# KubiakJakub01/Blokus-RL

Measured on AMD Instinct MI355X. Metric: MCTS sims/sec on 20x20 Blokus (4 players, 256 games/GPU, 100 sims/move), higher is better.
Workload: dtype fp32 net (fp32 operands split into f16 hi+lo, 3 f16 MFMA products, f32 accumulation: fp32-class error, tests/test_leafnet_gpu.py) / f64 search / u32 bitboards; 1 GPU; config 3 (N=1) / 4 (N=8): AlphaZero self-play 20x20, 256 concurrent games per GPU, 100 sims/move, ResNet-5x64 leaf eval; global_batch=256, parallelism=dp1 (independent games), model=resnet

## Files before the change

### blokus_rl_amd/alphazero/batched_mcts.py

```python
from __future__ import annotations

import ctypes

import numpy as np
import torch

from ..engine import Engine, EngineError, _check, _ptr


_OWN_OBS = object()


class BatchedMCTS:
    def __init__(self, eng: Engine, trees: int, node_cap: int = 8192, child_cap: int | None = None):
        self.eng = eng
        self.lib = eng.lib
        self.T = trees
        self.node_cap = node_cap
        if child_cap is None:
            per_node = 256 if eng.N >= 14 else 64
            child_cap = trees * node_cap * per_node
        self.child_cap = child_cap
        h = ctypes.c_void_p()
        with torch.cuda.device(eng.device):
# ... 46 lines not shown
        assert weight.is_contiguous() and weight.shape == (self.eng.A, feat.shape[1]) and bias.shape == (self.eng.A,)
        assert values.dtype == torch.float32 and values.shape == (self.T, self.eng.P)
        sel = roots is not None
        if obs is _OWN_OBS:
            obs = self.obs
        if obs is not None:
            assert obs.dtype == torch.float32 and obs.shape == self.obs.shape and obs.device == self.obs.device
        _check(self.lib.bk_mcts_leaf_step(self.h, ctypes.c_void_p(feat.data_ptr()), feat.stride(0), feat.shape[1],
                                          _ptr(weight), _ptr(bias), _ptr(values), int(sel), _ptr(roots),
                                          _ptr(active), float(cpuct), _ptr(self.status) if sel else None,
                                          _ptr(obs) if sel else None,
                                          _ptr(self.leaf_mask) if sel and want_mask else None,
                                          self._s()))
        return (self.status, obs, self.leaf_mask) if sel else None

    @property
    def leaf_states_ptr(self) -> int:
        p = ctypes.c_void_p()
        _check(self.lib.bk_mcts_leaf_states(self.h, ctypes.byref(p)))
        return int(p.value)

    def root_policy(self, roots: torch.Tensor, active: torch.Tensor | None, temperature: float, cap: int = 2048,
                    zero: bool = True):
        alloc = torch.zeros if zero else torch.empty
        ids = alloc((self.T, cap), dtype=torch.int32, device=self.eng.device)
        pi = alloc((self.T, cap), dtype=torch.float64, device=self.eng.device)
        counts = alloc(self.T, dtype=torch.int32, device=self.eng.device)
        _check(self.lib.bk_mcts_root_policy(self.h, _ptr(roots), _ptr(active), float(temperature), _ptr(ids),
                                            _ptr(pi), cap, _ptr(counts), self._s()))
        return ids, pi, counts
# ... 49 lines not shown
```

### blokus_rl_amd/alphazero/selfplay.py

```python
from __future__ import annotations

import os
import time
from dataclasses import dataclass, field

import torch

from ..engine import Engine, _check, _ptr
from .batched_mcts import BatchedMCTS


@dataclass
class Examples:
    states: torch.Tensor
    ids: torch.Tensor
    pi: torch.Tensor
    k: torch.Tensor
    z: torch.Tensor

    def __len__(self):
        return int(self.states.shape[0])


@dataclass
# ... 90 lines not shown
            return self.const_logp, self.const_v
        if self.graph is not None:
            if obs.data_ptr() != self.static_obs.data_ptr():
                self.static_obs.copy_(obs)
            self.graph.replay()
            return self.static_lp, self.static_v
        return self._forward(obs)


class SelfPlay:
    def __init__(self, eng: Engine, model: torch.nn.Module | None, games: int, num_sims: int = 100,
                 cpuct: float = 1.0, temperature: float = 1.0, dirichlet_alpha: float = 1.0,
                 dirichlet_weight: float = 0.25, node_cap: int | None = None, child_cap: int | None = None,
                 cap: int = 2048, seed: int = 0, nn_dtype: torch.dtype = torch.float32, use_graph: bool = True,
                 continuous: bool = False, sim_graph_sims: int | None = None, record_plies: int | None = None,
                 leaf_input: str | None = None):
        self.eng = eng
        self.G = games
        self.num_sims = num_sims
        self.sim_graph_sims = (sim_graph_sims or int(os.environ.get("BK_SIM_GRAPH_SIMS", "0"))
                               or self.graph_sims_for(num_sims))
        self.cpuct = cpuct
        self.temperature = temperature
        self.alpha = dirichlet_alpha
        self.weight = dirichlet_weight
        self.cap = cap
        self.continuous = continuous
        self.record_plies = record_plies if record_plies is not None else (
            4 * self.max_game_plies(eng) if continuous else 0)
        if node_cap is None:
            node_cap = self.node_cap_for(eng, num_sims)
        self.mcts = BatchedMCTS(eng, games, node_cap=node_cap, child_cap=child_cap)
        self.evaluator = LeafEvaluator(model, eng, games, nn_dtype, use_graph)
        self._use_graph = use_graph
        mode = leaf_input if leaf_input is not None else os.environ.get("BK_LEAF_INPUT", "planes")
        if mode not in ("planes", "states"):
            raise ValueError(f"leaf_input / BK_LEAF_INPUT must be planes or states, got {mode!r}")
        self.leaf_input = mode if mode == "planes" or self.evaluator.takes_states else "planes"
        if getattr(self.evaluator, "planar", False) and self.evaluator.graph is not None:
            self.mcts.obs = self.evaluator.static_obs
        dev = eng.device
        self.gen = torch.Generator(device=dev)
        self.gen.manual_seed(seed)
        self._seed = int(seed) & 0xFFFFFFFFFFFFFFFF
        self._init_state = eng.init_states(1)
        self.roots = eng.init_states(games)
        self.active = torch.ones(games, dtype=torch.int32, device=dev)
        self.first_ply = torch.ones(games, dtype=torch.bool, device=dev)
        self.game_id = torch.arange(games, dtype=torch.int64, device=dev)
        self._stats = SelfPlayStats()
        self._next_gid = torch.full((), games, dtype=torch.int64, device=dev)
        self._sims_dev = torch.zeros((), dtype=torch.int64, device=dev)
        self._fin_dev = torch.zeros((), dtype=torch.int64, device=dev)
        self._zcap = 0
        self.z_table = torch.zeros((0, eng.P), dtype=torch.float32, device=dev)
        self.z_known = torch.zeros(0, dtype=torch.bool, device=dev)
        self._ensure_zcap()
        self._records: list[tuple[torch.Tensor, ...]] = []
        self.timers = None
        self._graph = None
        self._window: list[tuple[torch.Tensor, ...]] = []
        self._dropped_plies = 0
        self._cap_overflow = torch.zeros((), dtype=torch.int32, device=dev)
        self.last_action = torch.full((games,), -1, dtype=torch.int32, device=dev)

    @staticmethod
    def max_game_plies(eng: Engine) -> int:
        return eng.num_pieces * eng.P

    @classmethod
    def node_cap_for(cls, eng: Engine, num_sims: int) -> int:
        return int(num_sims) * cls.max_game_plies(eng) + 1

    def check(self) -> dict:
        from ..engine import EngineError

        c = self.mcts.check()
        if int(self._cap_overflow.item()):
            raise EngineError(f"a root had more than cap={self.cap} children: raise SelfPlay(cap=...)")
# ... 20 lines not shown
            out, v = self.evaluator.forward_states(self.mcts.leaf_states_ptr, self.mcts.status)
        else:
            out, v = self.evaluator(obs)
        if self.evaluator.sparse:
            self.mcts.leaf_logits(out, self.evaluator.policy_w, self.evaluator.policy_b)
            return None, v, 2
        return out, v, 0

    def simulate(self):
        if self.timers is not None:
            return self._simulate_timed()
        _, obs, _ = self.mcts.select(self.roots, self.active, self.cpuct)
        logp, v, mode = self._evaluate(obs)
        self.mcts.expand_backup(logp, v, prior_mode=mode)


    @staticmethod
    def graph_sims_for(num_sims: int) -> int:
        if num_sims <= 100:
            return max(num_sims, 1)
        d = max(k for k in range(1, 101) if num_sims % k == 0)
        return d if d >= 10 else 10

    def _simulations(self, n: int):
        k = self.sim_graph_sims
        if n >= k and self._graph_usable():
            g = self._sim_graph()
            self._g_roots.copy_(self.roots)
            self._g_active.copy_(self.active)
            for _ in range(n // k):
                g.replay()
            n -= (n // k) * k
        for _ in range(n):
            self.simulate()

    def _graph_usable(self) -> bool:
        ev = self.evaluator
        return (self.timers is None and self._use_graph and (ev.model is None or ev.graph is not None)
                and os.environ.get("BK_SIM_GRAPH", "1") != "0")

    def _sim_body(self):
        _, obs, _ = self.mcts.select(self._g_roots, self._g_active, self.cpuct)
        ev = self.evaluator
        if ev.model is None:
            self.mcts.expand_backup(ev.const_logp, ev.const_v, prior_mode=0)
            return
        if self.leaf_input == "states":
            out, v = ev.forward_states(self.mcts.leaf_states_ptr, self.mcts.status)
        else:
            out, v = ev._forward(obs)
        if ev.sparse:
            self.mcts.leaf_logits(out, ev.policy_w, ev.policy_b)
            self.mcts.expand_backup(None, v, prior_mode=2)
        else:
            self.mcts.expand_backup(out, v, prior_mode=0)

    def _sim_graph(self):
        if self._graph is None:
            self._g_roots = self.roots.clone()
            self._g_active = self.active.clone()
            ev = self.evaluator
            g = torch.cuda.CUDAGraph()
            with torch.cuda.graph(g):
                if ev.model is not None and ev.sparse:
                    _, obs, _ = self.mcts.select(self._g_roots, self._g_active, self.cpuct)
                    states = self.leaf_input == "states"
                    for i in range(self.sim_graph_sims):
                        if states:
                            out, v = ev.forward_states(self.mcts.leaf_states_ptr, self.mcts.status)
                        else:
                            out, v = ev._forward(obs)
                        last = i == self.sim_graph_sims - 1
                        self.mcts.leaf_step(out, ev.policy_w, ev.policy_b, v, None if last else self._g_roots,
                                            self._g_active, self.cpuct, want_mask=False,
                                            obs=None if states else obs)
                else:
                    for _ in range(self.sim_graph_sims):
                        self._sim_body()
            self._graph = g
# ... 173 lines not shown
```

### blokus_rl_amd/csrc/mcts.hip

```cpp
#define BK_BOARD_SYNC() ::bk::wave_lds_sync()
#ifdef BK_STAMPS
#include <hip/hip_runtime.h>
static __device__ unsigned long long g_step_stamps[4096][16];
#define BK_MASK_STAMP(i) \
  do { if (threadIdx.x == 0 && blockIdx.x < 4096 && blockDim.x > 256) g_step_stamps[blockIdx.x][i] = __builtin_amdgcn_s_memtime(); } while (0)
#endif
#include <algorithm>
#include <cmath>
#include <cstring>
#include <vector>

#include "../../include/blokus_engine.h"
#include "ctx.h"
#include "legal_rows.h"
#include "mcts_dev.h"

namespace bk {

constexpr int kResetBlocks = 8;
__global__ __launch_bounds__(256) void k_reset(DevMcts m, const int32_t* flags) {
  const int t = blockIdx.y;
  if (flags && !flags[t]) return;
  TabEntry* tab = m.tab + (size_t)t * m.TS;
  for (int i = blockIdx.x * 256 + threadIdx.x; i < m.TS; i += kResetBlocks * 256) tab[i] = TabEntry{0ull, 0u, 0};
  if (blockIdx.x == 0 && threadIdx.x == 0) { m.tree_nodes[t] = 0; m.tree_children[t] = 0; }
}

constexpr int kSelectWaves = 4;
__global__ __launch_bounds__(64 * kSelectWaves) void k_select(DevPreset dp, DevMcts m, const uint32_t* __restrict__ roots,
                                                              const int32_t* __restrict__ active, double cpuct,
                                                              int32_t* __restrict__ status_out, float* __restrict__ obs,
                                                              uint64_t* __restrict__ mask_out, double root_eps) {
  extern __shared__ __attribute__((aligned(16))) uint32_t lds[];
  __shared__ int status_sh;
  const int wave = __builtin_amdgcn_readfirstlane(threadIdx.x >> 6);
  if (wave == 0) {
    const int st = select_descend(dp, m, blockIdx.x, roots, active, cpuct, status_out, lds, 0, nullptr, root_eps);
    if (lane_id() == 0) status_sh = st;
  }
  __syncthreads();
  select_leaf<kSelectWaves>(dp, m, blockIdx.x, status_sh, obs, mask_out, lds, wave);
}

constexpr int kLeafR = 1;
__global__ __launch_bounds__(256) void k_leaf_logits(DevPreset dp, DevMcts m, const float* __restrict__ feat,
                                                     int64_t ldf, int F, const float* __restrict__ W,
                                                     const float* __restrict__ bias) {
  extern __shared__ __attribute__((aligned(16))) uint32_t lds[];
  leaf_logits_tree<kLeafR>(dp, m, blockIdx.x, blockIdx.y, kLeafBlocks, feat, ldf, F, W, bias, lds);
}

__global__ __launch_bounds__(64) void k_expand_backup(DevPreset dp, DevMcts m, const float* __restrict__ logp,
                                                      const float* __restrict__ values, int prior_mode) {
  extern __shared__ __attribute__((aligned(16))) uint32_t lds[];
  expand_tree(dp, m, blockIdx.x, logp, values, prior_mode, lds);
}

__device__ __forceinline__ void wg_store_handoff() {
  __builtin_amdgcn_s_waitcnt(0x0F70);
  __syncthreads();
  asm volatile("buffer_inv sc0" ::: "memory");
}
constexpr int kStepWaves = 16;
__global__ __launch_bounds__(64 * kStepWaves) void k_leaf_step(DevPreset dp, DevMcts m, const float* __restrict__ feat,
                                                                 int64_t ldf, int F, const float* __restrict__ W,
                                                                 const float* __restrict__ bias,
                                                                 const float* __restrict__ values, int do_select,
                                                                 const uint32_t* __restrict__ roots,
                                                                 const int32_t* __restrict__ active, double cpuct,
                                                                 int32_t* __restrict__ status_out,
                                                                 float* __restrict__ obs,
                                                                 uint64_t* __restrict__ mask_out) {
  extern __shared__ __attribute__((aligned(16))) uint32_t lds[];
  __shared__ int status_sh;
  const int t = blockIdx.x;
  const int wave = __builtin_amdgcn_readfirstlane(threadIdx.x >> 6);
#ifdef BK_STAMPS
#define BK_STEP_STAMP(i) \
  do { if (do_select && threadIdx.x == 0 && t < 4096) g_step_stamps[t][i] = __builtin_amdgcn_s_memtime(); } while (0)
#else
#define BK_STEP_STAMP(i) do { } while (0)
#endif
  BK_STEP_STAMP(0);
  leaf_logits_tree<kLeafR>(dp, m, t, 0, 1, feat, ldf, F, W, bias, lds);
  wg_store_handoff();
  BK_STEP_STAMP(1);
  if (wave == 0) expand_tree(dp, m, t, nullptr, values, 2, lds);
  wg_store_handoff();
  BK_STEP_STAMP(2);
  if (!do_select) return;
// ... 5 lines not shown
  BK_STEP_STAMP(3);
  select_leaf<kStepWaves>(dp, m, t, status_sh, obs, mask_out, lds, wave);
  BK_STEP_STAMP(4);
#undef BK_STEP_STAMP
}

__global__ __launch_bounds__(64 * kStepWaves) void k_leaf_step_ov(DevPreset dp, DevMcts m, const float* __restrict__ feat,
                                                                    int64_t ldf, int F, const float* __restrict__ W,
                                                                    const float* __restrict__ bias,
                                                                    const float* __restrict__ values, int do_select,
                                                                    const uint32_t* __restrict__ roots,
                                                                    const int32_t* __restrict__ active, double cpuct,
                                                                    int32_t* __restrict__ status_out,
                                                                    float* __restrict__ obs,
                                                                    uint64_t* __restrict__ mask_out, int sel_off,
                                                                    int skipz) {
  extern __shared__ __attribute__((aligned(16))) uint32_t lds[];
  __shared__ int status_sh, status0_sh;
  __shared__ StepExpand sx;
  const int t = blockIdx.x;
  const int wave = __builtin_amdgcn_readfirstlane(threadIdx.x >> 6);
#ifdef BK_STAMPS
#define BK_OV_STAMP(i) \
  do { if (lane_id() == 0 && do_select && t < 4096) g_step_stamps[t][i] = __builtin_amdgcn_s_memtime(); } while (0)
#else
#define BK_OV_STAMP(i) do { } while (0)
#endif
  if (threadIdx.x == 0) {
    sx.ready = 0;
    sx.pready = 0;
    sx.done = 0;
    sx.leaf_ready = 0;
    sx.slice = 0;
    sx.loaded = 0;
    sx.counted = 0;
// ... 247 lines not shown
  if (!rc) rc = mcts_alloc(m, &d.tree_ctr, T * 8);
  if (!rc) rc = hip_check(hipMemset(d.tree_ctr, 0, T * 8 * sizeof(unsigned long long)), "memset tree counters");
  if (!rc) rc = hip_check(hipMemset(d.leaf_status, 0, T * sizeof(int32_t)), "memset status");
  if (!rc) rc = hip_check(hipMemset(d.depth, 0, T * sizeof(int32_t)), "memset depth");
  if (rc) { bk_mcts_destroy(m); return rc; }
  rc = bk_mcts_reset(m, nullptr, nullptr);
  if (!rc) rc = hip_check(hipDeviceSynchronize(), "sync");
  if (rc) { bk_mcts_destroy(m); return rc; }
  *out = m;
  return BK_OK;
}

int bk_mcts_destroy(bk_mcts* m) {
  if (!m) return BK_OK;
  for (void* p : m->allocs) (void)hipFree(p);
  delete m;
  return BK_OK;
}

int bk_mcts_reset(bk_mcts* m, const int32_t* reset_flags, void* stream) {
  BK_REQUIRE(m, "null mcts");
  hipLaunchKernelGGL(k_reset, dim3(kResetBlocks, m->d.T), dim3(256), 0, (hipStream_t)stream, m->d,
                     reset_flags);
  return launch_check("k_reset");
}

int bk_mcts_select_eps(bk_mcts* m, const void* roots, const int32_t* active, double cpuct, double root_eps,
                       int32_t* leaf_status, float* obs, uint64_t* leaf_mask, void* stream) {
  BK_REQUIRE(m && roots && leaf_status && obs, "bad argument");
  BK_REQUIRE(root_eps >= 0.0, "bk_mcts_select_eps: root_eps >= 0");
  const DevPreset& dp = m->ctx->dp;
  const size_t lds = sizeof(uint32_t) * (size_t)(kStateWords + 2 * kMaxN + dp.W32pad);
  hipLaunchKernelGGL(k_select, dim3(m->d.T), dim3(kWave * kSelectWaves), lds, (hipStream_t)stream, dp, m->d,
                     (const uint32_t*)roots, active, cpuct, leaf_status, obs, leaf_mask, root_eps);
  return launch_check("k_select");
}

int bk_mcts_select(bk_mcts* m, const void* roots, const int32_t* active, double cpuct, int32_t* leaf_status,
                   float* obs, uint64_t* leaf_mask, void* stream) {
  return bk_mcts_select_eps(m, roots, active, cpuct, 1e-6, leaf_status, obs, leaf_mask, stream);
}

int bk_mcts_leaf_logits(bk_mcts* m, const float* feat, int64_t ldf, int F, const float* W, const float* bias,
                        void* stream) {
  BK_REQUIRE(m && feat && W && bias && F > 0 && F <= kMaxFeat && ldf >= F, "bad argument");
  BK_REQUIRE(((uintptr_t)W & 15u) == 0 || (F & 3) != 0, "bk_mcts_leaf_logits: W must be 16-byte aligned");
  const DevPreset& dp = m->ctx->dp;
  const size_t lds = sizeof(uint32_t) * ((size_t)dp.W32pad + kLeafCap + F);
  hipLaunchKernelGGL(k_leaf_logits, dim3(m->d.T, kLeafBlocks), dim3(256), lds, (hipStream_t)stream, dp, m->d, feat,
                     ldf, F, W, bias);
  return launch_check("k_leaf_logits");
}

int bk_mcts_leaf_step(bk_mcts* m, const float* feat, int64_t ldf, int F, const float* W, const float* bias,
                      const float* values, int do_select, const void* roots, const int32_t* active, double cpuct,
                      int32_t* leaf_status, float* obs, uint64_t* leaf_mask, void* stream) {
  BK_REQUIRE(m && feat && W && bias && values && F > 0 && F <= kMaxFeat && ldf >= F, "bad argument");
  BK_REQUIRE(((uintptr_t)W & 15u) == 0 || (F & 3) != 0, "bk_mcts_leaf_step: W must be 16-byte aligned");
  BK_REQUIRE(!do_select || (roots && leaf_status), "bad argument: select outputs");
  const DevPreset& dp = m->ctx->dp;
  const char* ov = getenv("BK_STEP_OVERLAP");
  const int overlap = ov ? atoi(ov) : 1;
  if (overlap) {
    const int sel_off = (int)(((size_t)dp.W32pad + 2 * kLeafCap + F + 3) & ~(size_t)3);
    const size_t words = (size_t)sel_off + kStateWords + 2 * kMaxN + dp.W32pad;
    const char* sz = getenv("BK_LEAF_SKIP0");
    const int skipz = sz ? atoi(sz) : 1;
    hipLaunchKernelGGL(k_leaf_step_ov, dim3(m->d.T), dim3(kWave * kStepWaves), sizeof(uint32_t) * words,
                       (hipStream_t)stream, dp, m->d, feat, ldf, F, W, bias, values, do_select,
                       (const uint32_t*)roots, active, cpuct, leaf_status, obs, leaf_mask, sel_off, skipz);
    return launch_check("k_leaf_step_ov");
  }
  size_t words = (size_t)dp.W32pad + kLeafCap + F;
  words = std::max(words, (size_t)dp.W32pad + kExpandLdsIds);
  words = std::max(words, (size_t)(kStateWords + 2 * kMaxN + dp.W32pad));
  hipLaunchKernelGGL(k_leaf_step, dim3(m->d.T), dim3(kWave * kStepWaves), sizeof(uint32_t) * words,
                     (hipStream_t)stream, dp, m->d, feat, ldf, F, W, bias, values, do_select,
                     (const uint32_t*)roots, active, cpuct, leaf_status, obs, leaf_mask);
  return launch_check("k_leaf_step");
}

int bk_mcts_expand_backup(bk_mcts* m, const float* logp, const float* values, int prior_mode, void* stream) {
  BK_REQUIRE(m && values && (prior_mode == 0 || prior_mode == 1 || prior_mode == 2), "bad argument");
  BK_REQUIRE(logp || prior_mode == 2, "bad argument: logp");
  const DevPreset& dp = m->ctx->dp;
  const size_t lds = sizeof(uint32_t) * ((size_t)dp.W32pad + kExpandLdsIds);
  hipLaunchKernelGGL(k_expand_backup, dim3(m->d.T), dim3(kWave), lds, (hipStream_t)stream, dp, m->d, logp, values,
                     prior_mode);
  return launch_check("k_expand_backup");
}

int bk_mcts_root_policy(bk_mcts* m, const void* roots, const int32_t* active, double temperature, int32_t* ids,
                        double* pi, int cap, int32_t* counts, void* stream) {
  BK_REQUIRE(m && roots && ids && pi && counts && cap > 0 && temperature >= 0.0, "bad argument");
// ... 61 lines not shown
```

### blokus_rl_amd/csrc/mcts_dev.h

```cpp
#pragma once
#include <cmath>
#include <vector>

#include "../../include/blokus_engine.h"
#include "ctx.h"
#include "legal_rows.h"

namespace bk {

constexpr int kMaxDepth = 96;
constexpr int kExpandLdsIds = 2048;
constexpr int kGatherRegs = 16;
constexpr int kLeafCap = 2048;
constexpr int kLeafBlocks = 4;
constexpr int kMaxFeat = 2048;
constexpr int kLeafQ = 16;

#ifdef BK_STAMPS
static __device__ unsigned long long g_stamps[2][4096][8];
#define BK_STAMP(k, i) \
  do { if (lane_id() == 0 && blockIdx.x < 4096) g_stamps[k][blockIdx.x][i] = __builtin_amdgcn_s_memtime(); } while (0)
#else
#define BK_STAMP(k, i) do { } while (0)
#endif
// ... 924 lines not shown
  }
  for (int i = l + kGatherRegs * kWave; i < K; i += kWave) {
    m.ch_id[off + i] = ids[i];
    m.ch_N[off + i] = 0u;
    m.ch_Q[off + i] = 0.0;
    m.ch_P[off + i] = expf((lg[i] - mx) - lse);
  }
}

}

struct bk_mcts {
  bk_ctx* ctx = nullptr;
  bk::DevMcts d{};
  std::vector<void*> allocs;
};
```

### blokus_rl_amd/engine.py

```python
from __future__ import annotations

import ctypes
import os
from dataclasses import dataclass

import numpy as np
import torch

HERE = os.path.dirname(os.path.abspath(__file__))
LIB_PATH = os.environ.get("BK_LIB") or os.path.join(HERE, "_lib", "libblokus_hip.so")
STATE_BYTES = 384
STATE_WORDS = STATE_BYTES // 4

W_PIECES, W_HASH, W_TO_MOVE, W_PLY, W_FLAGS = 80, 84, 86, 87, 88

_vp = ctypes.c_void_p
_i = ctypes.c_int
_SIGS = {
    "bk_last_error": (ctypes.c_char_p, []),
    "bk_version": (_i, []),
    "bk_state_bytes": (_i, []),
    "bk_ctx_create": (_i, [_i, _i, _i, _i, ctypes.POINTER(_vp)]),
    "bk_ctx_destroy": (_i, [_vp]),
    "bk_action_size": (_i, [_vp]),
# ... 5 lines not shown
    "bk_legal_mask": (_i, [_vp, _vp, _vp, _i, _vp, _vp, _vp]),
    "bk_legal_ids": (_i, [_vp, _vp, _vp, _i, _vp, _i, _vp, _vp]),
    "bk_next_state": (_i, [_vp, _vp, _vp, _i, _vp, _vp, _vp, _vp]),
    "bk_game_ended": (_i, [_vp, _vp, _i, _vp, _vp, _vp]),
    "bk_observe": (_i, [_vp, _vp, _i, _vp, _vp]),
    "bk_square_counts": (_i, [_vp, _vp, _i, _vp, _vp]),
    "bk_mcts_create": (_i, [_vp, _i, _i, ctypes.c_int64, ctypes.POINTER(_vp)]),
    "bk_mcts_destroy": (_i, [_vp]),
    "bk_mcts_reset": (_i, [_vp, _vp, _vp]),
    "bk_mcts_select": (_i, [_vp, _vp, _vp, ctypes.c_double, _vp, _vp, _vp, _vp]),
    "bk_mcts_select_eps": (_i, [_vp, _vp, _vp, ctypes.c_double, ctypes.c_double, _vp, _vp, _vp, _vp]),
    "bk_mcts_expand_backup": (_i, [_vp, _vp, _vp, _i, _vp]),
    "bk_mcts_leaf_logits": (_i, [_vp, _vp, ctypes.c_int64, _i, _vp, _vp, _vp]),
    "bk_mcts_leaf_step": (_i, [_vp, _vp, ctypes.c_int64, _i, _vp, _vp, _vp, _i, _vp, _vp, ctypes.c_double, _vp,
                               _vp, _vp, _vp]),
    "bk_mcts_root_policy": (_i, [_vp, _vp, _vp, ctypes.c_double, _vp, _vp, _i, _vp, _vp]),
    "bk_mcts_root_stats": (_i, [_vp, _vp, _vp, _vp, _vp, _vp, _vp, _i, _vp, _vp]),
    "bk_mcts_counters": (_i, [_vp, _vp, _vp]),
    "bk_mcts_leaf_info": (_i, [_vp, _vp, _vp, _vp]),
    "bk_mcts_leaf_states": (_i, [_vp, ctypes.POINTER(_vp)]),
    "bk_ply_policy": (_i, [_vp, _vp, _vp, _vp, _vp, _i, _i, ctypes.c_double, ctypes.c_double, ctypes.c_uint64,
                           ctypes.c_uint64, _vp, _vp, _vp, _vp, _vp, _vp, _vp]),
    "bk_ply_finish": (_i, [_i, _i, _vp, _vp, _vp, _vp, _vp, _vp, _vp, _i, _i, _vp, _vp, _vp, _vp, _vp, _vp, _vp,
                           ctypes.c_int64, _vp, _vp, _vp, _vp, _vp]),
    "bk_vec_reset": (_i, [_vp, _vp, _vp, _vp, _i, _vp, _vp, _vp]),
    "bk_vec_step": (_i, [_vp, _vp, _vp, _vp, _i, _vp, _vp, _vp, _vp, _vp]),
    "bk_vec_policy": (_i, [_vp, _vp, _vp, _vp, _i, _i, _vp, _vp, _vp]),
    "bk_vec_step_policy": (_i, [_vp, _vp, _vp, _vp, _i, _i, _vp, _vp, _vp, _vp, _vp, _vp, _vp]),
    "bk_replay_stride": (ctypes.c_size_t, [_i]),
    "bk_replay_batch": (_i, [_vp, _vp, _i, _vp, _i, _vp, _vp, _vp, _vp, _vp, _vp, _vp]),
# ... 32 lines not shown
    "bk_resnet_stem_tower_heads": (_i, [_vp, _i, _i, _i, _vp, _vp, _i, _vp, _vp, _vp, _vp, _vp, _vp, _vp, _vp, _vp,
                                        _vp, _vp, _vp, _vp, _vp, _i, _vp, _vp, _vp]),
    "bk_leafnet_x3_weight_bytes": (_i, [_i]),
    "bk_leafnet_x3_supported": (_i, [_i]),
    "bk_leafnet_x3": (_i, [_vp, _i, _i, _i, _vp, _vp, _vp, _i, _vp, _vp, _vp, _vp] + [_vp] * 8 + [_i, _vp, _vp, _vp, _vp]),
    "bk_leafnet_x3_states": (_i, [_vp, _vp, _i, _i, _i, _vp, _vp, _vp, _i, _vp, _vp, _vp, _vp] + [_vp] * 8
                             + [_vp, _vp, _vp, _vp]),
    "bk_leafnet_w3_weight_bytes": (_i, []),
    "bk_leafnet_w3_supported": (_i, [_i]),
    "bk_leafnet_w3": (_i, [_vp, _i, _i, _i, _vp, _vp, _vp, _i, _vp, _vp, _vp, _vp] + [_vp] * 8 + [_i, _vp, _vp, _vp, _vp, _vp]),
}

_LIB = None


class EngineError(RuntimeError):
    pass


def load_library(path: str = LIB_PATH) -> ctypes.CDLL:
    global _LIB
    if _LIB is not None:
        return _LIB
    if not os.path.exists(path):
        raise EngineError(
            f"HIP engine library not built: {path}. Run `python -c 'import __graft_entry__ as g; g.build()'`."
        )
    lib = ctypes.CDLL(path)
    for name, (res, args) in _SIGS.items():
        fn = getattr(lib, name)
# ... 184 lines not shown
```

### blokus_rl_amd/nets.py

```python
from __future__ import annotations

import ctypes

import torch
import torch.nn.functional as F
from torch import nn


class NativeBatchNorm2d(nn.BatchNorm2d):

    def forward(self, x):
        self._check_input_dim(x)
        factor = 0.0 if self.momentum is None else self.momentum
        if self.training and self.track_running_stats and self.num_batches_tracked is not None:
            self.num_batches_tracked.add_(1)
            factor = 1.0 / float(self.num_batches_tracked) if self.momentum is None else self.momentum
        use_batch = self.training or (self.running_mean is None and self.running_var is None)
        track = not self.training or self.track_running_stats
        rm = self.running_mean if track else None
        rv = self.running_var if track else None
        return torch.native_batch_norm(x, self.weight, self.bias, rm, rv, use_batch, factor, self.eps)[0]


def use_native_batchnorm(model: nn.Module) -> nn.Module:
# ... 315 lines not shown
    nl = 2 * len(f.blocks)
    assert model.x3_wtower.numel() == nl * lib.bk_leafnet_x3_weight_bytes(64)
    assert model.x3_wstem.numel() == lib.bk_leafnet_x3_weight_bytes(8)
    P = f.value_fc2.out_features
    pf = torch.empty((B, 2 * N * N), dtype=torch.float32, device=dev)
    v = torch.empty((B, P), dtype=torch.float32, device=dev)
    out = torch.empty((B, 64, N, N), dtype=torch.float32, device=dev,
                      memory_format=torch.channels_last) if want_out else None
    h = model.x3_heads
    _check(lib.bk_leafnet_x3_states(
        sptr, _ptr(status), B, N, f.stem.in_channels // 2, _ptr(model.x3_wstem), _ptr(model.x3_sstem), _ptr(h[0]), nl,
        _ptr(model.x3_wtower), _ptr(model.x3_stower), _ptr(model.b_tower), _ptr(model.x3_bounds),
        *[_ptr(t) for t in h[1:]], _ptr(pf), _ptr(v),
        None if out is None else ctypes.c_void_p(out.data_ptr()), _stream(dev)))
    return (pf, v, out) if want_out else (pf, v)


_OBSERVERS: dict = {}


def _observe_states(states: torch.Tensor, N: int, P: int) -> torch.Tensor:
    from .engine import Engine

    key = (N, P, states.device)
    eng = _OBSERVERS.get(key)
    if eng is None:
        eng = _OBSERVERS[key] = Engine(N, P, 5, device=states.device)
    return eng.observe(states.contiguous())


# ... 256 lines not shown
```

### include/blokus_engine.h

```cpp
#ifndef BLOKUS_ENGINE_H
#define BLOKUS_ENGINE_H

#include <stddef.h>
#include <stdint.h>

#ifdef __cplusplus
extern "C" {
#endif

#define BK_OK 0
#define BK_EINVAL -1
#define BK_EHIP -2
#define BK_EILLEGAL -3
#define BK_ECAPACITY -4
#define BK_ENOMEM -5

#define BK_STATE_BYTES 384
#define BK_MAX_N 20
#define BK_MAX_P 4

typedef struct bk_ctx bk_ctx;
typedef struct bk_mcts bk_mcts;

const char* bk_last_error(void);
// ... 32 lines not shown

int bk_mcts_select(bk_mcts* m, const void* roots, const int32_t* active, double cpuct,
                   int32_t* leaf_status, float* obs, uint64_t* leaf_mask, void* stream);
int bk_mcts_select_eps(bk_mcts* m, const void* roots, const int32_t* active, double cpuct, double root_eps,
                       int32_t* leaf_status, float* obs, uint64_t* leaf_mask, void* stream);

int bk_mcts_expand_backup(bk_mcts* m, const float* logp, const float* values, int prior_mode,
                          void* stream);

int bk_mcts_leaf_logits(bk_mcts* m, const float* feat, int64_t ldf, int F, const float* W, const float* bias,
                        void* stream);

int bk_mcts_leaf_step(bk_mcts* m, const float* feat, int64_t ldf, int F, const float* W, const float* bias,
                      const float* values, int do_select, const void* roots, const int32_t* active, double cpuct,
                      int32_t* leaf_status, float* obs, uint64_t* leaf_mask, void* stream);

int bk_mcts_root_policy(bk_mcts* m, const void* roots, const int32_t* active, double temperature,
                        int32_t* ids, double* pi, int cap, int32_t* counts, void* stream);

int bk_mcts_root_stats(bk_mcts* m, const void* roots, const int32_t* active, int32_t* ids,
                       uint32_t* n, double* q, float* p, int cap, int32_t* counts, void* stream);

int bk_mcts_leaf_info(bk_mcts* m, void* leaf_states, int32_t* depths, void* stream);

int bk_mcts_leaf_states(bk_mcts* m, const void** states);

int bk_mcts_counters(bk_mcts* m, int64_t* out, void* stream);

int bk_ply_policy(const int32_t* ids, const double* pi, const int32_t* counts, const int32_t* active,
                  const uint8_t* first_ply, int G, int cap, double dirichlet_weight, double dirichlet_alpha,
// ... 96 lines not shown

int bk_leafnet_x3_states(const void* states, const int32_t* status, int B, int N, int P, const void* wstem,
                         const float* sstem, const float* bstem, int nlayers, const void* wtower,
                         const float* stower, const float* btower, const float* bounds, const float* wp,
                         const float* bp, const float* wv, const float* bv, const float* w1t, const float* b1,
                         const float* w2, const float* b2, float* pf, float* vout, float* out, void* stream);

int bk_leafnet_w3_weight_bytes(void);
int bk_leafnet_w3_supported(int N);
int bk_leafnet_w3(const float* obs, int B, int N, int cin, const void* wstem, const float* sstem, const float* bstem,
                  int nlayers, const void* utower, const float* stower, const float* btower, const float* bounds,
                  const float* wp, const float* bp, const float* wv, const float* bv, const float* w1t, const float* b1,
                  const float* w2, const float* b2, int P, float* pf, float* vout, float* x0ws, float* out,
                  void* stream);

#ifdef __cplusplus
}
#endif
#endif
```

Before: 1.330 million sims/s.

## Pipeline MCTS simulations across game groups on multiple streams

Splits the trees into up to four groups, each on its own HIP stream. Each group runs its own select, leaf-net and leaf-step chain, linked by ring events, so tree-search kernels of one group can overlap the network evaluation of another inside the captured graph. Kernels gain a t0 offset so they can run on a subrange of trees. This adds stream and event management and more, smaller launches. It is on by default (4 groups) when the evaluator is sparse fp32 and takes states.

New measurement: 1.442 million sims/s, median of 6. 8.4% higher.

```diff
diff --git a/blokus_rl_amd/alphazero/batched_mcts.py b/blokus_rl_amd/alphazero/batched_mcts.py
--- a/blokus_rl_amd/alphazero/batched_mcts.py
+++ b/blokus_rl_amd/alphazero/batched_mcts.py
@@ -84,6 +84,34 @@
                                           self._s()))
         return (self.status, obs, self.leaf_mask) if sel else None
 
+    def select_range(self, t0: int, n: int, roots: torch.Tensor, active: torch.Tensor | None, cpuct: float = 1.0):
+        _check(self.lib.bk_mcts_select_range(self.h, int(t0), int(n), _ptr(roots), _ptr(active), float(cpuct),
+                                             _ptr(self.status), _ptr(self.obs), _ptr(self.leaf_mask), self._s()))
+        return self.status, self.obs, self.leaf_mask
+
+    def leaf_step_range(self, t0: int, n: int, feat: torch.Tensor, weight: torch.Tensor, bias: torch.Tensor,
+                        values: torch.Tensor, roots: torch.Tensor | None = None, active: torch.Tensor | None = None,
+                        cpuct: float = 1.0):
+        assert feat.dtype == torch.float32 and feat.shape[0] == self.T and feat.stride(1) == 1
+        assert weight.is_contiguous() and weight.shape == (self.eng.A, feat.shape[1]) and bias.shape == (self.eng.A,)
+        assert values.dtype == torch.float32 and values.shape == (self.T, self.eng.P)
+        sel = roots is not None
+        _check(self.lib.bk_mcts_leaf_step_range(self.h, int(t0), int(n), ctypes.c_void_p(feat.data_ptr()),
+                                                feat.stride(0), feat.shape[1], _ptr(weight), _ptr(bias), _ptr(values),
+                                                int(sel), _ptr(roots), _ptr(active), float(cpuct),
+                                                _ptr(self.status) if sel else None, _ptr(self.obs) if sel else None,
+                                                _ptr(self.leaf_mask) if sel else None, self._s()))
+        return (self.status, self.obs, self.leaf_mask) if sel else None
+
+    def sims_pipelined(self, net_args, n_sims: int, groups: int, weight: torch.Tensor, bias: torch.Tensor,
+                       roots: torch.Tensor, active: torch.Tensor | None, cpuct: float = 1.0,
+                       obs: torch.Tensor | None = None, ring: int = 1):
+        assert weight.is_contiguous() and bias.shape == (self.eng.A,)
+        assert weight.shape == (self.eng.A, 2 * self.eng.N * self.eng.N)
+        _check(self.lib.bk_mcts_sims_pipelined(self.h, ctypes.byref(net_args), int(n_sims), int(groups), int(ring),
+                                               _ptr(weight), _ptr(bias), _ptr(roots), _ptr(active), float(cpuct),
+                                               _ptr(self.status), _ptr(obs), self._s()))
+
     @property
     def leaf_states_ptr(self) -> int:
         p = ctypes.c_void_p()
diff --git a/blokus_rl_amd/alphazero/selfplay.py b/blokus_rl_amd/alphazero/selfplay.py
--- a/blokus_rl_amd/alphazero/selfplay.py
+++ b/blokus_rl_amd/alphazero/selfplay.py
@@ -128,7 +128,8 @@
                  dirichlet_weight: float = 0.25, node_cap: int | None = None, child_cap: int | None = None,
                  cap: int = 2048, seed: int = 0, nn_dtype: torch.dtype = torch.float32, use_graph: bool = True,
                  continuous: bool = False, sim_graph_sims: int | None = None, record_plies: int | None = None,
-                 leaf_input: str | None = None):
+                 leaf_input: str | None = None, sim_groups: int | None = None, sim_ring: int | bool | None = None,
+                 sim_groups_min_games: int = 64):
         self.eng = eng
         self.G = games
         self.num_sims = num_sims
@@ -153,6 +154,17 @@
         self.leaf_input = mode if mode == "planes" or self.evaluator.takes_states else "planes"
         if getattr(self.evaluator, "planar", False) and self.evaluator.graph is not None:
             self.mcts.obs = self.evaluator.static_obs
+        k = int(sim_groups if sim_groups is not None else os.environ.get("BK_SIM_GROUPS", self.SIM_GROUPS_DEFAULT))
+        if k not in (1, 2, 4):
+            raise ValueError(f"sim_groups / BK_SIM_GROUPS must be 1, 2 or 4, got {k}")
+        ev = self.evaluator
+        pipelined = (ev.sparse and ev.dtype == torch.float32 and ev.model.takes_states()
+                     and games >= max(sim_groups_min_games, k))
+        self.sim_groups = k if pipelined else 1
+        ring = sim_ring if sim_ring is not None else os.environ.get("BK_SIM_RING")
+        self.sim_ring = int(ring) if ring is not None else (1 if self.sim_groups == 2 else 2)
+        if self.sim_ring not in (0, 1, 2):
+            raise ValueError(f"sim_ring / BK_SIM_RING must be 0, 1 or 2, got {self.sim_ring}")
         dev = eng.device
         self.gen = torch.Generator(device=dev)
         self.gen.manual_seed(seed)
@@ -173,10 +185,13 @@
         self._records: list[tuple[torch.Tensor, ...]] = []
         self.timers = None
         self._graph = None
+        self._pipe_args = None
         self._window: list[tuple[torch.Tensor, ...]] = []
         self._dropped_plies = 0
         self._cap_overflow = torch.zeros((), dtype=torch.int32, device=dev)
         self.last_action = torch.full((games,), -1, dtype=torch.int32, device=dev)
+
+    SIM_GROUPS_DEFAULT = 4
 
     @staticmethod
     def max_game_plies(eng: Engine) -> int:
@@ -227,6 +242,23 @@
         logp, v, mode = self._evaluate(obs)
         self.mcts.expand_backup(logp, v, prior_mode=mode)
 
+    def _pipelined(self, n: int, roots: torch.Tensor, active: torch.Tensor, eager: bool = False):
+        if self._pipe_args is None:
+            from ..nets import leafnet_x3_args
+
+            ev, m, N = self.evaluator, self.mcts, self.eng.N
+            states = self.leaf_input == "states"
+            pf = torch.empty((self.G, 2 * N * N), dtype=torch.float32, device=self.eng.device)
+            v = torch.empty((self.G, self.eng.P), dtype=torch.float32, device=self.eng.device)
+            args = leafnet_x3_args(ev.model, pf, v, obs=None if states else m.obs,
+                                   states=m.leaf_states_ptr if states else None, status=m.status if states else None)
+            self._pipe_args = (args, pf, v, None if states else m.obs)
+        args, _, _, obs = self._pipe_args
+        ev = self.evaluator
+        groups, ring = (min(self.sim_groups, 2), 1) if eager else (self.sim_groups, self.sim_ring)
+        self.mcts.sims_pipelined(args, n, groups, ev.policy_w, ev.policy_b, roots, active, self.cpuct, obs=obs,
+                                 ring=ring)
+
 
     @staticmethod
     def graph_sims_for(num_sims: int) -> int:
@@ -244,6 +276,9 @@
             for _ in range(n // k):
                 g.replay()
             n -= (n // k) * k
+        elif n > 0 and self.sim_groups > 1 and self.timers is None:
+            self._pipelined(n, self.roots, self.active, eager=True)
+            n = 0
         for _ in range(n):
             self.simulate()
 
@@ -273,9 +308,13 @@
             self._g_roots = self.roots.clone()
             self._g_active = self.active.clone()
             ev = self.evaluator
+            if self.sim_groups > 1:
+                self._pipelined(0, self._g_roots, self._g_active)
             g = torch.cuda.CUDAGraph()
             with torch.cuda.graph(g):
-                if ev.model is not None and ev.sparse:
+                if self.sim_groups > 1:
+                    self._pipelined(self.sim_graph_sims, self._g_roots, self._g_active)
+                elif ev.model is not None and ev.sparse:
                     _, obs, _ = self.mcts.select(self._g_roots, self._g_active, self.cpuct)
                     states = self.leaf_input == "states"
                     for i in range(self.sim_graph_sims):
diff --git a/blokus_rl_amd/csrc/mcts.hip b/blokus_rl_amd/csrc/mcts.hip
--- a/blokus_rl_amd/csrc/mcts.hip
+++ b/blokus_rl_amd/csrc/mcts.hip
@@ -30,16 +30,17 @@
 __global__ __launch_bounds__(64 * kSelectWaves) void k_select(DevPreset dp, DevMcts m, const uint32_t* __restrict__ roots,
                                                               const int32_t* __restrict__ active, double cpuct,
                                                               int32_t* __restrict__ status_out, float* __restrict__ obs,
-                                                              uint64_t* __restrict__ mask_out, double root_eps) {
+                                                              uint64_t* __restrict__ mask_out, double root_eps, int t0) {
   extern __shared__ __attribute__((aligned(16))) uint32_t lds[];
   __shared__ int status_sh;
+  const int t = t0 + blockIdx.x;
   const int wave = __builtin_amdgcn_readfirstlane(threadIdx.x >> 6);
   if (wave == 0) {
-    const int st = select_descend(dp, m, blockIdx.x, roots, active, cpuct, status_out, lds, 0, nullptr, root_eps);
+    const int st = select_descend(dp, m, t, roots, active, cpuct, status_out, lds, 0, nullptr, root_eps);
     if (lane_id() == 0) status_sh = st;
   }
   __syncthreads();
-  select_leaf<kSelectWaves>(dp, m, blockIdx.x, status_sh, obs, mask_out, lds, wave);
+  select_leaf<kSelectWaves>(dp, m, t, status_sh, obs, mask_out, lds, wave);
 }
 
 constexpr int kLeafR = 1;
@@ -70,10 +71,10 @@
                                                                  const int32_t* __restrict__ active, double cpuct,
                                                                  int32_t* __restrict__ status_out,
                                                                  float* __restrict__ obs,
-                                                                 uint64_t* __restrict__ mask_out) {
+                                                                 uint64_t* __restrict__ mask_out, int t0) {
   extern __shared__ __attribute__((aligned(16))) uint32_t lds[];
   __shared__ int status_sh;
-  const int t = blockIdx.x;
+  const int t = t0 + blockIdx.x;
   const int wave = __builtin_amdgcn_readfirstlane(threadIdx.x >> 6);
 #ifdef BK_STAMPS
 #define BK_STEP_STAMP(i) \
@@ -109,11 +110,11 @@
                                                                     int32_t* __restrict__ status_out,
                                                                     float* __restrict__ obs,
                                                                     uint64_t* __restrict__ mask_out, int sel_off,
-                                                                    int skipz) {
+                                                                    int skipz, int t0) {
   extern __shared__ __attribute__((aligned(16))) uint32_t lds[];
   __shared__ int status_sh, status0_sh;
   __shared__ StepExpand sx;
-  const int t = blockIdx.x;
+  const int t = t0 + blockIdx.x;
   const int wave = __builtin_amdgcn_readfirstlane(threadIdx.x >> 6);
 #ifdef BK_STAMPS
 #define BK_OV_STAMP(i) \
@@ -391,6 +392,13 @@
 int bk_mcts_destroy(bk_mcts* m) {
   if (!m) return BK_OK;
   for (void* p : m->allocs) (void)hipFree(p);
+  for (hipStream_t s : m->pipe_stream)
+    if (s) (void)hipStreamDestroy(s);
+  for (hipEvent_t e : m->pipe_step)
+    if (e) (void)hipEventDestroy(e);
+  for (hipEvent_t e : m->pipe_join)
+    if (e) (void)hipEventDestroy(e);
+  if (m->pipe_fork) (void)hipEventDestroy(m->pipe_fork);
   delete m;
   return BK_OK;
 }
@@ -402,20 +410,33 @@
   return launch_check("k_reset");
 }
 
+static int select_launch(bk_mcts* m, int t0, int n, const void* roots, const int32_t* active, double cpuct,
+                         double root_eps, int32_t* leaf_status, float* obs, uint64_t* leaf_mask, void* stream) {
+  if (n == 0) return BK_OK;
+  const DevPreset& dp = m->ctx->dp;
+  const size_t lds = sizeof(uint32_t) * (size_t)(kStateWords + 2 * kMaxN + dp.W32pad);
+  hipLaunchKernelGGL(k_select, dim3(n), dim3(kWave * kSelectWaves), lds, (hipStream_t)stream, dp, m->d,
+                     (const uint32_t*)roots, active, cpuct, leaf_status, obs, leaf_mask, root_eps, t0);
+  return launch_check("k_select");
+}
+
 int bk_mcts_select_eps(bk_mcts* m, const void* roots, const int32_t* active, double cpuct, double root_eps,
                        int32_t* leaf_status, float* obs, uint64_t* leaf_mask, void* stream) {
   BK_REQUIRE(m && roots && leaf_status && obs, "bad argument");
   BK_REQUIRE(root_eps >= 0.0, "bk_mcts_select_eps: root_eps >= 0");
-  const DevPreset& dp = m->ctx->dp;
-  const size_t lds = sizeof(uint32_t) * (size_t)(kStateWords + 2 * kMaxN + dp.W32pad);
-  hipLaunchKernelGGL(k_select, dim3(m->d.T), dim3(kWave * kSelectWaves), lds, (hipStream_t)stream, dp, m->d,
-                     (const uint32_t*)roots, active, cpuct, leaf_status, obs, leaf_mask, root_eps);
-  return launch_check("k_select");
+  return select_launch(m, 0, m->d.T, roots, active, cpuct, root_eps, leaf_status, obs, leaf_mask, stream);
 }
 
 int bk_mcts_select(bk_mcts* m, const void* roots, const int32_t* active, double cpuct, int32_t* leaf_status,
                    float* obs, uint64_t* leaf_mask, void* stream) {
   return bk_mcts_select_eps(m, roots, active, cpuct, 1e-6, leaf_status, obs, leaf_mask, stream);
+}
+
+int bk_mcts_select_range(bk_mcts* m, int t0, int n, const void* roots, const int32_t* active, double cpuct,
+                         int32_t* leaf_status, float* obs, uint64_t* leaf_mask, void* stream) {
+  BK_REQUIRE(m && roots && leaf_status && obs, "bk_mcts_select_range: bad argument");
+  BK_REQUIRE(t0 >= 0 && n >= 0 && (int64_t)t0 + n <= m->d.T, "bk_mcts_select_range: need 0 <= t0, 0 <= n, t0 + n <= T");
+  return select_launch(m, t0, n, roots, active, cpuct, 1e-6, leaf_status, obs, leaf_mask, stream);
 }
 
 int bk_mcts_leaf_logits(bk_mcts* m, const float* feat, int64_t ldf, int F, const float* W, const float* bias,
@@ -429,12 +450,11 @@
   return launch_check("k_leaf_logits");
 }
 
-int bk_mcts_leaf_step(bk_mcts* m, const float* feat, int64_t ldf, int F, const float* W, const float* bias,
-                      const float* values, int do_select, const void* roots, const int32_t* active, double cpuct,
-                      int32_t* leaf_status, float* obs, uint64_t* leaf_mask, void* stream) {
-  BK_REQUIRE(m && feat && W && bias && values && F > 0 && F <= kMaxFeat && ldf >= F, "bad argument");
-  BK_REQUIRE(((uintptr_t)W & 15u) == 0 || (F & 3) != 0, "bk_mcts_leaf_step: W must be 16-byte aligned");
-  BK_REQUIRE(!do_select || (roots && leaf_status), "bad argument: select outputs");
+static int leaf_step_launch(bk_mcts* m, int t0, int n, const float* feat, int64_t ldf, int F, const float* W,
+                            const float* bias, const float* values, int do_select, const void* roots,
+                            const int32_t* active, double cpuct, int32_t* leaf_status, float* obs,
+                            uint64_t* leaf_mask, void* stream) {
+  if (n == 0) return BK_OK;
   const DevPreset& dp = m->ctx->dp;
   const char* ov = getenv("BK_STEP_OVERLAP");
   const int overlap = ov ? atoi(ov) : 1;
@@ -443,18 +463,129 @@
     const size_t words = (size_t)sel_off + kStateWords + 2 * kMaxN + dp.W32pad;
     const char* sz = getenv("BK_LEAF_SKIP0");
     const int skipz = sz ? atoi(sz) : 1;
-    hipLaunchKernelGGL(k_leaf_step_ov, dim3(m->d.T), dim3(kWave * kStepWaves), sizeof(uint32_t) * words,
+    hipLaunchKernelGGL(k_leaf_step_ov, dim3(n), dim3(kWave * kStepWaves), sizeof(uint32_t) * words,
                        (hipStream_t)stream, dp, m->d, feat, ldf, F, W, bias, values, do_select,
-                       (const uint32_t*)roots, active, cpuct, leaf_status, obs, leaf_mask, sel_off, skipz);
+                       (const uint32_t*)roots, active, cpuct, leaf_status, obs, leaf_mask, sel_off, skipz, t0);
     return launch_check("k_leaf_step_ov");
   }
   size_t words = (size_t)dp.W32pad + kLeafCap + F;
   words = std::max(words, (size_t)dp.W32pad + kExpandLdsIds);
   words = std::max(words, (size_t)(kStateWords + 2 * kMaxN + dp.W32pad));
-  hipLaunchKernelGGL(k_leaf_step, dim3(m->d.T), dim3(kWave * kStepWaves), sizeof(uint32_t) * words,
+  hipLaunchKernelGGL(k_leaf_step, dim3(n), dim3(kWave * kStepWaves), sizeof(uint32_t) * words,
                      (hipStream_t)stream, dp, m->d, feat, ldf, F, W, bias, values, do_select,
-                     (const uint32_t*)roots, active, cpuct, leaf_status, obs, leaf_mask);
+                     (const uint32_t*)roots, active, cpuct, leaf_status, obs, leaf_mask, t0);
   return launch_check("k_leaf_step");
+}
+
+int bk_mcts_leaf_step(bk_mcts* m, const float* feat, int64_t ldf, int F, const float* W, const float* bias,
+                      const float* values, int do_select, const void* roots, const int32_t* active, double cpuct,
+                      int32_t* leaf_status, float* obs, uint64_t* leaf_mask, void* stream) {
+  BK_REQUIRE(m && feat && W && bias && values && F > 0 && F <= kMaxFeat && ldf >= F, "bad argument");
+  BK_REQUIRE(((uintptr_t)W & 15u) == 0 || (F & 3) != 0, "bk_mcts_leaf_step: W must be 16-byte aligned");
+  BK_REQUIRE(!do_select || (roots && leaf_status), "bad argument: select outputs");
+  return leaf_step_launch(m, 0, m->d.T, feat, ldf, F, W, bias, values, do_select, roots, active, cpuct, leaf_status,
+                          obs, leaf_mask, stream);
+}
+
+int bk_mcts_leaf_step_range(bk_mcts* m, int t0, int n, const float* feat, int64_t ldf, int F, const float* W,
+                            const float* bias, const float* values, int do_select, const void* roots,
+                            const int32_t* active, double cpuct, int32_t* leaf_status, float* obs,
+                            uint64_t* leaf_mask, void* stream) {
+  BK_REQUIRE(m && feat && W && bias && values && F > 0 && F <= kMaxFeat && ldf >= F,
+             "bk_mcts_leaf_step_range: bad argument");
+  BK_REQUIRE(((uintptr_t)W & 15u) == 0 || (F & 3) != 0, "bk_mcts_leaf_step_range: W must be 16-byte aligned");
+  BK_REQUIRE(!do_select || (roots && leaf_status), "bk_mcts_leaf_step_range: bad argument: select outputs");
+  BK_REQUIRE(t0 >= 0 && n >= 0 && (int64_t)t0 + n <= m->d.T,
+             "bk_mcts_leaf_step_range: need 0 <= t0, 0 <= n, t0 + n <= T");
+  return leaf_step_launch(m, t0, n, feat, ldf, F, W, bias, values, do_select, roots, active, cpuct, leaf_status, obs,
+                          leaf_mask, stream);
+}
+
+static int pipe_prepare(bk_mcts* m) {
+  if (m->pipe_ready) return BK_OK;
+  int rc = hip_check(hipSetDevice(m->ctx->device), "hipSetDevice");
+  for (int g = 0; !rc && g < bk_mcts::kMaxGroups - 1; ++g) {
+    if (!m->pipe_stream[g])
+      rc = hip_check(hipStreamCreateWithFlags(&m->pipe_stream[g], hipStreamNonBlocking), "create group stream");
+    if (!rc && !m->pipe_join[g])
+      rc = hip_check(hipEventCreateWithFlags(&m->pipe_join[g], hipEventDisableTiming), "create join event");
+  }
+  for (int g = 0; !rc && g < bk_mcts::kMaxGroups; ++g)
+    if (!m->pipe_step[g])
+      rc = hip_check(hipEventCreateWithFlags(&m->pipe_step[g], hipEventDisableTiming), "create step event");
+  if (!rc && !m->pipe_fork) rc = hip_check(hipEventCreateWithFlags(&m->pipe_fork, hipEventDisableTiming), "create fork event");
+  if (!rc) m->pipe_ready = true;
+  return rc;
+}
+
+static int pipe_net(const bk_leafnet_args* a, int t0, int n, void* stream) {
+  const size_t F = (size_t)2 * a->N * a->N;
+  float* pf = a->pf + (size_t)t0 * F;
+  float* vout = a->vout + (size_t)t0 * a->P;
+  if (a->states)
+    return bk_leafnet_x3_states((const char*)a->states + (size_t)t0 * kStateBytes, a->status ? a->status + t0 : nullptr,
+                                n, a->N, a->P, a->wstem, a->sstem, a->bstem, a->nlayers, a->wtower, a->stower,
+                                a->btower, a->bounds, a->wp, a->bp, a->wv, a->bv, a->w1t, a->b1, a->w2, a->b2, pf,
+                                vout, nullptr, stream);
+  return bk_leafnet_x3(a->obs + (size_t)t0 * 2 * a->P * a->N * a->N, n, a->N, 2 * a->P, a->wstem, a->sstem, a->bstem,
+                       a->nlayers, a->wtower, a->stower, a->btower, a->bounds, a->wp, a->bp, a->wv, a->bv, a->w1t,
+                       a->b1, a->w2, a->b2, a->P, pf, vout, nullptr, stream);
+}
+
+int bk_mcts_sims_pipelined(bk_mcts* m, const bk_leafnet_args* net, int n_sims, int groups, int ring, const float* W,
+                           const float* bias, const void* roots, const int32_t* active, double cpuct,
+                           int32_t* leaf_status, float* obs, void* stream) {
+  BK_REQUIRE(m && net && W && bias && roots && leaf_status, "bk_mcts_sims_pipelined: bad argument");
+  BK_REQUIRE(groups == 1 || groups == 2 || groups == 4, "bk_mcts_sims_pipelined: groups must be 1, 2 or 4");
+  BK_REQUIRE(n_sims >= 0, "bk_mcts_sims_pipelined: n_sims >= 0");
+  BK_REQUIRE(ring >= 0 && ring <= 2, "bk_mcts_sims_pipelined: ring must be 0, 1 or 2");
+  BK_REQUIRE((net->obs != nullptr) != (net->states != nullptr),
+             "bk_mcts_sims_pipelined: the net reads either obs or states");
+  BK_REQUIRE(!net->obs || obs == net->obs, "bk_mcts_sims_pipelined: the search must write the planes the net reads");
+  BK_REQUIRE(!net->states || net->status == leaf_status,
+             "bk_mcts_sims_pipelined: the net must read the status the search writes");
+  BK_REQUIRE(net->pf && net->vout && net->P > 0 && net->P <= kMaxP && net->N > 0 && net->N <= kMaxN,
+             "bk_mcts_sims_pipelined: bad net arguments");
+  const int F = 2 * net->N * net->N;
+  BK_REQUIRE(F <= kMaxFeat, "bk_mcts_sims_pipelined: too many policy features");
+  BK_REQUIRE(((uintptr_t)W & 15u) == 0 || (F & 3) != 0, "bk_mcts_sims_pipelined: W must be 16-byte aligned");
+  int rc = pipe_prepare(m);
+  if (rc || n_sims == 0) return rc;
+  const int T = m->d.T;
+  const int per = (T + groups - 1) / groups;
+  const int G = (T + per - 1) / per;
+  hipStream_t st[bk_mcts::kMaxGroups];
+  st[0] = (hipStream_t)stream;
+  for (int g = 1; g < G; ++g) st[g] = m->pipe_stream[g - 1];
+  int forked = 1;
+  if (G > 1) rc = hip_check(hipEventRecord(m->pipe_fork, st[0]), "record fork");
+  for (int g = 1; !rc && g < G; ++g) {
+    rc = hip_check(hipStreamWaitEvent(st[g], m->pipe_fork, 0), "fork group stream");
+    if (!rc) forked = g + 1;
+  }
+  const auto n_of = [&](int g) { return std::min(T, (g + 1) * per) - g * per; };
+  for (int g = 0; !rc && g < G; ++g)
+    rc = select_launch(m, g * per, n_of(g), roots, active, cpuct, 1e-6, leaf_status, obs, nullptr, st[g]);
+  for (int g = 0; !rc && g < G; ++g) rc = pipe_net(net, g * per, n_of(g), st[g]);
+  for (int s = 0; !rc && s < n_sims; ++s) {
+    const int do_select = s + 1 < n_sims;
+    const bool edges = G > 1 && (ring == 1 || (ring == 2 && s == 0));
+    for (int g = 0; !rc && g < G; ++g) {
+      if (edges && (g > 0 || s > 0))
+        rc = hip_check(hipStreamWaitEvent(st[g], m->pipe_step[g > 0 ? g - 1 : G - 1], 0), "ring edge");
+      if (!rc)
+        rc = leaf_step_launch(m, g * per, n_of(g), net->pf, F, F, W, bias, net->vout, do_select, roots, active, cpuct,
+                              leaf_status, obs, nullptr, st[g]);
+      if (!rc && edges) rc = hip_check(hipEventRecord(m->pipe_step[g], st[g]), "record step");
+      if (!rc && do_select) rc = pipe_net(net, g * per, n_of(g), st[g]);
+    }
+  }
+  for (int g = 1; g < forked; ++g) {
+    int rj = hip_check(hipEventRecord(m->pipe_join[g - 1], st[g]), "record join");
+    if (!rj) rj = hip_check(hipStreamWaitEvent(st[0], m->pipe_join[g - 1], 0), "join group stream");
+    if (!rc) rc = rj;
+  }
+  return rc;
 }
 
 int bk_mcts_expand_backup(bk_mcts* m, const float* logp, const float* values, int prior_mode, void* stream) {
diff --git a/blokus_rl_amd/csrc/mcts_dev.h b/blokus_rl_amd/csrc/mcts_dev.h
--- a/blokus_rl_amd/csrc/mcts_dev.h
+++ b/blokus_rl_amd/csrc/mcts_dev.h
@@ -962,4 +962,8 @@
   bk_ctx* ctx = nullptr;
   bk::DevMcts d{};
   std::vector<void*> allocs;
+  static constexpr int kMaxGroups = 4;
+  bool pipe_ready = false;
+  hipStream_t pipe_stream[kMaxGroups - 1] = {};
+  hipEvent_t pipe_fork = nullptr, pipe_step[kMaxGroups] = {}, pipe_join[kMaxGroups - 1] = {};
 };
diff --git a/blokus_rl_amd/engine.py b/blokus_rl_amd/engine.py
--- a/blokus_rl_amd/engine.py
+++ b/blokus_rl_amd/engine.py
@@ -43,6 +43,10 @@
     "bk_mcts_leaf_logits": (_i, [_vp, _vp, ctypes.c_int64, _i, _vp, _vp, _vp]),
     "bk_mcts_leaf_step": (_i, [_vp, _vp, ctypes.c_int64, _i, _vp, _vp, _vp, _i, _vp, _vp, ctypes.c_double, _vp,
                                _vp, _vp, _vp]),
+    "bk_mcts_select_range": (_i, [_vp, _i, _i, _vp, _vp, ctypes.c_double, _vp, _vp, _vp, _vp]),
+    "bk_mcts_leaf_step_range": (_i, [_vp, _i, _i, _vp, ctypes.c_int64, _i, _vp, _vp, _vp, _i, _vp, _vp,
+                                     ctypes.c_double, _vp, _vp, _vp, _vp]),
+    "bk_mcts_sims_pipelined": (_i, [_vp, _vp, _i, _i, _i, _vp, _vp, _vp, _vp, ctypes.c_double, _vp, _vp, _vp]),
     "bk_mcts_root_policy": (_i, [_vp, _vp, _vp, ctypes.c_double, _vp, _vp, _i, _vp, _vp]),
     "bk_mcts_root_stats": (_i, [_vp, _vp, _vp, _vp, _vp, _vp, _vp, _i, _vp, _vp]),
     "bk_mcts_counters": (_i, [_vp, _vp, _vp]),
@@ -105,6 +109,12 @@
 _LIB = None
 
 
+class LeafnetArgs(ctypes.Structure):
+    _fields_ = ([("obs", _vp), ("states", _vp), ("status", _vp), ("N", _i), ("P", _i), ("nlayers", _i)]
+                + [(k, _vp) for k in ("wstem", "sstem", "bstem", "wtower", "stower", "btower", "bounds", "wp", "bp",
+                                      "wv", "bv", "w1t", "b1", "w2", "b2", "pf", "vout")])
+
+
 class EngineError(RuntimeError):
     pass
 
diff --git a/blokus_rl_amd/nets.py b/blokus_rl_amd/nets.py
--- a/blokus_rl_amd/nets.py
+++ b/blokus_rl_amd/nets.py
@@ -353,6 +353,40 @@
         *[_ptr(t) for t in h[1:]], _ptr(pf), _ptr(v),
         None if out is None else ctypes.c_void_p(out.data_ptr()), _stream(dev)))
     return (pf, v, out) if want_out else (pf, v)
+
+
+def leafnet_x3_args(model: "LeafResNet", pf: torch.Tensor, v: torch.Tensor, obs: torch.Tensor | None = None,
+                    states=None, status: torch.Tensor | None = None):
+    from .engine import LeafnetArgs, load_library
+
+    assert (obs is None) != (states is None)
+    f = model.f
+    lib = load_library()
+    N, P, nl = model.board_size, f.value_fc2.out_features, 2 * len(f.blocks)
+    assert model.x3 and f.stem.in_channels == 2 * P and lib.bk_leafnet_x3_supported(N)
+    assert model.x3_wtower.numel() == nl * lib.bk_leafnet_x3_weight_bytes(64)
+    assert model.x3_wstem.numel() == lib.bk_leafnet_x3_weight_bytes(8)
+    B = pf.shape[0]
+    dev = model.x3_wstem.device
+    for t, shape in ((pf, (B, 2 * N * N)), (v, (B, P))):
+        assert t.dtype == torch.float32 and t.shape == shape and t.is_contiguous() and t.device == dev
+    a = LeafnetArgs()
+    if obs is not None:
+        assert obs.dtype == torch.float32 and obs.shape == (B, 2 * P, N, N) and obs.is_contiguous() and obs.device == dev
+        a.obs = obs.data_ptr()
+    else:
+        assert status is not None and status.dtype == torch.int32 and status.shape == (B,) and status.device == dev
+        a.states = states.data_ptr() if isinstance(states, torch.Tensor) else int(states)
+        a.status = status.data_ptr()
+    a.N, a.P, a.nlayers = N, P, nl
+    h = model.x3_heads
+    tensors = {"wstem": model.x3_wstem, "sstem": model.x3_sstem, "bstem": h[0], "wtower": model.x3_wtower,
+               "stower": model.x3_stower, "btower": model.b_tower, "bounds": model.x3_bounds, "pf": pf, "vout": v}
+    tensors.update(zip(("wp", "bp", "wv", "bv", "w1t", "b1", "w2", "b2"), h[1:]))
+    for k, t in tensors.items():
+        assert t.is_contiguous() and t.device == dev
+        setattr(a, k, t.data_ptr())
+    return a
 
 
 _OBSERVERS: dict = {}
diff --git a/include/blokus_engine.h b/include/blokus_engine.h
--- a/include/blokus_engine.h
+++ b/include/blokus_engine.h
@@ -70,6 +70,13 @@
 int bk_mcts_leaf_step(bk_mcts* m, const float* feat, int64_t ldf, int F, const float* W, const float* bias,
                       const float* values, int do_select, const void* roots, const int32_t* active, double cpuct,
                       int32_t* leaf_status, float* obs, uint64_t* leaf_mask, void* stream);
+
+int bk_mcts_select_range(bk_mcts* m, int t0, int n, const void* roots, const int32_t* active, double cpuct,
+                         int32_t* leaf_status, float* obs, uint64_t* leaf_mask, void* stream);
+int bk_mcts_leaf_step_range(bk_mcts* m, int t0, int n, const float* feat, int64_t ldf, int F, const float* W,
+                            const float* bias, const float* values, int do_select, const void* roots,
+                            const int32_t* active, double cpuct, int32_t* leaf_status, float* obs,
+                            uint64_t* leaf_mask, void* stream);
 
 int bk_mcts_root_policy(bk_mcts* m, const void* roots, const int32_t* active, double temperature,
                         int32_t* ids, double* pi, int cap, int32_t* counts, void* stream);
@@ -196,6 +203,34 @@
                   const float* w2, const float* b2, int P, float* pf, float* vout, float* x0ws, float* out,
                   void* stream);
 
+typedef struct bk_leafnet_args {
+  const float* obs;
+  const void* states;
+  const int32_t* status;
+  int N, P, nlayers;
+  const void* wstem;
+  const float* sstem;
+  const float* bstem;
+  const void* wtower;
+  const float* stower;
+  const float* btower;
+  const float* bounds;
+  const float* wp;
+  const float* bp;
+  const float* wv;
+  const float* bv;
+  const float* w1t;
+  const float* b1;
+  const float* w2;
+  const float* b2;
+  float* pf;
+  float* vout;
+} bk_leafnet_args;
+
+int bk_mcts_sims_pipelined(bk_mcts* m, const bk_leafnet_args* net, int n_sims, int groups, int ring, const float* W,
+                           const float* bias, const void* roots, const int32_t* active, double cpuct,
+                           int32_t* leaf_status, float* obs, void* stream);
+
 #ifdef __cplusplus
 }
 #endif
```
